# Fangjin98/distributed-training-INA

Hardware: AMD Instinct MI355X
Metric: aggregated-gradient GB/s (device-resident), 8-worker×100 MB int32 sum-reduce (higher is better)
Workload: dtype int32; 1 GPU; C3: 8 workers x 100 MiB int32 (26,214,400 values), V=256 slots; workers=8, slots=102400

## Files before the change

### distributed-training-ina_amd/csrc/ina_switch.hip

```cpp
#include <hip/hip_runtime.h>

#include <algorithm>
#include <atomic>
#include <cmath>
#include <mutex>
#include <unordered_map>

#include "ina.h"
#include "ina_internal.h"
#include "ina_device.h"

namespace ina {

using u32x4s = u32x4_t;
using f32x4s = f32x4_t;

constexpr int kSwBlock = 256;
constexpr int kMaxV = 256;
constexpr int kMaxStride = 16 + 4 * kMaxV;

__device__ __forceinline__ uint32_t from_next_lane(uint32_t x) {
    return (uint32_t)__builtin_amdgcn_update_dpp((int)x, (int)x, 0x130, 0xF, 0xF, false);
}
__device__ __forceinline__ uint32_t from_prev_lane(uint32_t x) {
// ... 614 lines not shown
#pragma unroll
    for (int o = 1; o < 64; o <<= 1) {
        const uint32_t y = (uint32_t)__shfl_up((int)x, o);
        if (lane >= o) x = max(x, y);
    }
    return x;
}
__device__ __forceinline__ uint32_t wave_suffix_min(uint32_t x) {
    const int lane = threadIdx.x & 63;
#pragma unroll
    for (int o = 1; o < 64; o <<= 1) {
        const uint32_t y = (uint32_t)__shfl_down((int)x, o);
        if (lane + o < 64) x = min(x, y);
    }
    return x;
}

#ifndef INA_LOC_TIMING
#define INA_LOC_TIMING 0
#endif
#if INA_LOC_TIMING
__device__ unsigned long long g_loc_t[8192][4];
#define LOC_STAMP(q) do { if (threadIdx.x == 0 && u < 8192) g_loc_t[u][q] = wall_clock64(); } while (0)
#define DEC_STAMP(row, q) do { if (threadIdx.x == 0) g_loc_t[row][q] = wall_clock64(); } while (0)
#else
#define LOC_STAMP(q) do { } while (0)
#define DEC_STAMP(row, q) do { } while (0)
#endif

struct LocUnit {
    uint32_t g_lo, lo, hi, pad;
};

__device__ __forceinline__ bool local_decide(const uint32_t* __restrict__ gmin, const uint32_t* __restrict__ gmax,
                                             uint32_t G, uint32_t gsize, size_t npk,
                                             uint32_t* __restrict__ unsorted, uint32_t epoch,
                                             LocUnit* __restrict__ units, bool writer, uint32_t* s_pm,
                                             uint32_t* s_sm, uint32_t* s_a, uint32_t* s_b) {
    __shared__ unsigned long long s_cost[kBkWaves];
    const int lane = threadIdx.x & 63, wv = wave_in_block();
    constexpr int kGpt = kLocMaxGran / kBkThr;
    const uint32_t kpt = (G + kBkThr - 1) / kBkThr;
    const uint32_t g0 = threadIdx.x * kpt;
    uint32_t pm[kGpt], sm[kGpt];
#pragma unroll
    for (int j = 0; j < kGpt; ++j) {
        const uint32_t g = g0 + (uint32_t)j;
        const bool ok = (uint32_t)j < kpt && g < G;
        pm[j] = ok ? gmax[g] : 0u;
        sm[j] = ok ? gmin[g] : 0xFFFFFFFFu;
    }
    uint32_t tmax = 0, tmin = 0xFFFFFFFFu;
#pragma unroll
    for (int j = 0; j < kGpt; ++j) pm[j] = tmax = max(tmax, pm[j]);
#pragma unroll
    for (int j = kGpt - 1; j >= 0; --j) sm[j] = tmin = min(tmin, sm[j]);
    const uint32_t imx = wave_incl_max(tmax), imn = wave_suffix_min(tmin);
    if (lane == 63) s_a[wv] = imx;
    if (lane == 0) s_b[wv] = imn;
    __syncthreads();
    uint32_t xmx = 0, xmn = 0xFFFFFFFFu, kmax = 0, kmin = 0xFFFFFFFFu;
#pragma unroll
    for (int w = 0; w < kBkWaves; ++w) {
        const uint32_t a = s_a[w], b = s_b[w];
        xmx = w < wv ? max(xmx, a) : xmx;
        xmn = w > wv ? min(xmn, b) : xmn;
        kmax = max(kmax, a);
        kmin = min(kmin, b);
    }
    {
        const uint32_t up = (uint32_t)__shfl_up((int)imx, 1), dn = (uint32_t)__shfl_down((int)imn, 1);
        if (lane > 0) xmx = max(xmx, up);
        if (lane < 63) xmn = min(xmn, dn);
    }
#pragma unroll
    for (int j = 0; j < kGpt; ++j) {
        const uint32_t g = g0 + (uint32_t)j;
        if ((uint32_t)j < kpt && g < G) {
            s_pm[g] = max(pm[j], xmx);
            s_sm[g] = min(sm[j], xmn);
        }
    }
    __syncthreads();
    if (kmin > kmax) return false;
    DEC_STAMP(8189, 0);
    constexpr uint32_t kUpt = (kLocMaxGran / kLocU + kBkThr - 1) / kBkThr;
    const uint32_t nu = (G + kLocU - 1) / kLocU;
    const uint32_t upt = (nu + kBkThr - 1) / kBkThr;
    LocUnit mu[kUpt];
    unsigned long long cost = 0;
    uint32_t maxwin = 0, glo = 0;
#pragma unroll
    for (uint32_t j = 0; j < kUpt; ++j) {
        const uint32_t u = threadIdx.x * upt + j;
        mu[j] = LocUnit{0u, 0u, 0u, 0u};
        if (j >= upt || u >= nu) continue;
        const uint32_t a = s_sm[u * kLocU];
        const uint32_t b = (u + 1) * kLocU < G ? s_sm[(u + 1) * kLocU] : 0xFFFFFFFFu;
        const uint32_t lo = a == 0xFFFFFFFFu ? kmax + 1u : a, hi = b == 0xFFFFFFFFu ? kmax + 1u : b;
        uint32_t l = glo, r = G;
        if (j > 0)
            for (int s = 0; s < 8 && l < r && s_pm[l] < lo; ++s) ++l;
        if (l < r && s_pm[l] < lo)
            while (l < r) {
                const uint32_t m = (l + r) >> 1;
                if (s_pm[m] >= lo) r = m; else l = m + 1;
            }
        glo = l;
        mu[j] = LocUnit{l, lo, hi, 0u};
        const size_t p0 = (size_t)l * gsize, p1 = min((size_t)(u + 1) * kLocU * gsize, npk);
        const uint32_t win = hi > lo && p1 > p0 ? (uint32_t)min(p1 - p0, (size_t)0xFFFFFFFFu) : 0u;
        cost += (unsigned long long)((hi - lo + kLlBins - 1) / kLlBins) * win;
        maxwin = max(maxwin, win);
    }
    DEC_STAMP(8189, 1);
#pragma unroll
    for (int o = 32; o > 0; o >>= 1) {
        cost += (unsigned long long)__shfl_xor((long long)cost, o);
        maxwin = max(maxwin, (uint32_t)__shfl_xor((int)maxwin, o));
    }
    if (lane == 0) {
        s_cost[wv] = cost;
        s_a[wv] = maxwin;
    }
    __syncthreads();
    unsigned long long total = 0;
    uint32_t mw = 0;
#pragma unroll
    for (int w = 0; w < kBkWaves; ++w) {
        total += s_cost[w];
        mw = max(mw, s_a[w]);
    }
    DEC_STAMP(8189, 2);
    if (mw > kLocMaxWindow || total > (unsigned long long)kLocBeta * npk) return false;
    if (writer) {
#pragma unroll
        for (uint32_t j = 0; j < kUpt; ++j) {
            const uint32_t u = threadIdx.x * upt + j;
            if (j < upt && u < nu) units[u] = mu[j];
        }
        if (threadIdx.x == 0) {
            unsorted[kLocKmin] = kmin;
            unsorted[kLocSlots] = kmax + 1u - kmin;
            unsorted[kLocUnits] = nu;
            unsorted[kLocEpoch] = epoch;
        }
    }
    return true;
}


__device__ __forceinline__ size_t switch_block_index();
__device__ __forceinline__ size_t xcd_block_index();
#ifndef INA_LL_WAVES_PER_EU
#define INA_LL_WAVES_PER_EU 8
#endif
__global__ __launch_bounds__(kLlWaves * 64) __attribute__((amdgpu_waves_per_eu(INA_LL_WAVES_PER_EU, 8))) void k_local_lists(const KeySrc keys_in, size_t npk,
                                                               uint32_t num_slots, uint32_t kmask,
                                                               const uint32_t* __restrict__ unsorted,
                                                               const LocUnit* __restrict__ units, uint32_t gsize,
                                                               uint32_t* __restrict__ ids, uint2* __restrict__ tab) {
    constexpr int kThr = kLlWaves * 64;
    constexpr int DPT = kLlBins / kThr;
    __shared__ uint32_t cw[kLlWaves / 2][kLlBins];
    __shared__ uint32_t s_ws[kLlWaves];
    const uint32_t ep = unsorted[1];
    if (unsorted[kLocEpoch] != ep) return;
    KeySrc kall = keys_in;
    kall.epoch = ep;
    const int lane = threadIdx.x & 63, wv = wave_in_block();
    const int sh = (wv & 1) * 16;
    uint32_t* crow = cw[wv >> 1];
    const unsigned long long below = (1ull << lane) - 1ull;
    const uint32_t kmin = unsorted[kLocKmin], nunits = unsorted[kLocUnits];
    for (uint32_t u = (uint32_t)xcd_block_index(); u < nunits; u += gridDim.x) {
        const LocUnit w = units[u];
        if (w.hi <= w.lo) continue;
        LOC_STAMP(0);
        const uint32_t P0 = w.g_lo * gsize, Pu = u * kLocU * gsize;
        const uint32_t P1 = (uint32_t)min((size_t)Pu + (size_t)kLocU * gsize, npk);
        const uint32_t per = ((P1 - P0 + kLlWaves * 64 - 1) / (kLlWaves * 64)) * 64;
        const uint32_t b0 = min(P0 + (uint32_t)wv * per, P1), b1 = min(b0 + per, P1);
        const bool held = per <= 64u * kLlRounds;
        KeySrc keys = kall;
        if (kall.desc && kall.flags) {
            bool miss = false;
            for (uint32_t f = (P0 >> kall.kb_shift) + (uint32_t)lane; f <= ((P1 - 1u) >> kall.kb_shift); f += 64u)
                miss |= kall.flags[f] != ep;
            if (__ballot(miss)) keys.flags = nullptr;
            else keys.desc = nullptr;
        }
        uint32_t kk[kLlRounds];
        if (held) {
#pragma unroll
            for (int r = 0; r < kLlRounds; ++r) {
                const uint32_t p = b0 + (uint32_t)(r * 64 + lane);
                kk[r] = p < b1 ? keys(p) : num_slots;
            }
        }
        uint32_t area = 0;
        for (uint32_t q = w.lo; q < w.hi; q += kLlBins) {
            const uint32_t qn = min((uint32_t)kLlBins, w.hi - q);
            for (uint32_t d = lane; d < (uint32_t)kLlBins; d += 64) crow[d] = 0u;
            __syncthreads();
            uint32_t before = 0;
            for (uint32_t r0 = b0; r0 < b1; r0 += 64 * kLlRounds) {
                if (!held) {
#pragma unroll
                    for (int r = 0; r < kLlRounds; ++r) {
                        const uint32_t p = r0 + (uint32_t)(r * 64 + lane);
                        kk[r] = p < b1 ? keys(p) : num_slots;
                    }
                }
#pragma unroll
                for (int r = 0; r < kLlRounds; ++r) {
                    const uint32_t slot = kk[r] & kmask;
                    const uint32_t p = r0 + (uint32_t)(r * 64 + lane);
                    lds_count_half(crow, slot - q, slot < num_slots && slot - q < qn, sh);
                    before += (p < Pu && p < b1 && (slot < w.lo || slot >= num_slots)) ? 1u : 0u;
                }
            }
            if (q == w.lo) {
#pragma unroll
                for (int o = 32; o > 0; o >>= 1) before += (uint32_t)__shfl_xor((int)before, o);
                if (lane == 0) s_ws[wv] = before;
            }
            __syncthreads();
            if (q == w.lo) {
                area = P0;
#pragma unroll
                for (int v = 0; v < kLlWaves; ++v) area += s_ws[v];
            }
            LOC_STAMP(1);
            uint32_t tc[DPT], tt = 0;
#pragma unroll
            for (int j = 0; j < DPT; ++j) {
                const uint32_t d = threadIdx.x * DPT + (uint32_t)j;
                uint32_t t = 0;
#pragma unroll
                for (int v2 = 0; v2 < kLlWaves / 2; ++v2) {
                    const uint32_t word = cw[v2][d];
                    t += (word & 0xFFFFu) + (word >> 16);
                }
                tc[j] = t;
                tt += t;
            }
            __syncthreads();
            const uint32_t inc = wave_incl_scan(tt);
            if (lane == 63) s_ws[wv] = inc;
            __syncthreads();
            uint32_t e = inc - tt, passn = 0;
#pragma unroll
            for (int v = 0; v < kLlWaves; ++v) {
                const uint32_t x = s_ws[v];
                e += v < wv ? x : 0u;
                passn += x;
            }
#pragma unroll
            for (int j = 0; j < DPT; ++j) {
                const uint32_t d = threadIdx.x * DPT + (uint32_t)j;
                if (d < qn) tab[q + d - kmin] = uint2{area + e, tc[j]};
                uint32_t b = e;
#pragma unroll
                for (int v2 = 0; v2 < kLlWaves / 2; ++v2) {
                    const uint32_t word = cw[v2][d];
                    const uint32_t lo16 = word & 0xFFFFu;
                    cw[v2][d] = b | ((b + lo16) << 16);
                    b += lo16 + (word >> 16);
                }
                e += tc[j];
            }
            __syncthreads();
            LOC_STAMP(2);
            for (uint32_t r0 = b0; r0 < b1; r0 += 64 * kLlRounds) {
                if (!held) {
#pragma unroll
                    for (int r = 0; r < kLlRounds; ++r) {
                        const uint32_t p = r0 + (uint32_t)(r * 64 + lane);
                        kk[r] = p < b1 ? keys(p) : num_slots;
                    }
                }
#pragma unroll
                for (int r = 0; r < kLlRounds; ++r) {
                    if (r0 + (uint32_t)(r * 64) >= b1) break;
                    const uint32_t slot = kk[r] & kmask;
                    const uint32_t d = slot - q;
                    const bool valid = slot < num_slots && d < qn;
                    const unsigned long long pm = lanes_with_digit(d, kLlBits, valid);
                    if (valid) {
                        const uint32_t rank = (uint32_t)__builtin_popcountll(pm & below);
                        const uint32_t cur = (crow[d] >> sh) & 0xFFFFu;
                        ids[area + cur + rank] = (r0 + (uint32_t)(r * 64 + lane)) | (kk[r] & ~kmask);
                        if (rank == 0) atomicAdd(&crow[d], (uint32_t)__builtin_popcountll(pm) << sh);
                    }
                }
            }
            area += passn;
            __syncthreads();
        }
        LOC_STAMP(3);
    }
}

#ifndef INA_SORT_STAGE_ALIAS
#define INA_SORT_STAGE_ALIAS 1
#endif
#ifndef INA_SORT_STAGE_MAX_R
#define INA_SORT_STAGE_MAX_R 8
#endif
#ifndef INA_SORT_STAGE
#define INA_SORT_STAGE 1
#endif
template <int R, int BINS, bool kStage = false, bool kPosOnly = false>
__device__ __forceinline__ void rs_tile_scatter_half(const uint32_t (&k)[R], const uint32_t (&v)[R],
                                                     size_t i0, size_t n, int shift, int bits,
                                                     uint32_t (*base)[BINS], const uint32_t* gst,
                                                     uint32_t* __restrict__ kout,
                                                     uint32_t* __restrict__ vout, int rw = R,
                                                     uint32_t* sk = nullptr, uint32_t* sv = nullptr,
                                                     uint32_t sbase = 0u, uint32_t* spos_out = nullptr) {
    const int lane = threadIdx.x & 63, wv = wave_in_block();
    const int sh = (wv & 1) * 16;
    uint32_t* row = base[wv >> 1];
    const uint32_t nb = 1u << bits;
    constexpr int kDPT = (BINS + kBkThr - 1) / kBkThr;
#pragma unroll
    for (int j = 0; j < kDPT; ++j) {
        const uint32_t d = threadIdx.x + (uint32_t)j * kBkThr;
        if (d >= nb) continue;
        uint32_t b = 0;
#pragma unroll
        for (int w2 = 0; w2 < kBkWaves / 2; ++w2) {
            const uint32_t word = base[w2][d];
            const uint32_t lo = word & 0xFFFFu, hi = word >> 16;
            base[w2][d] = b | ((b + lo) << 16);
            b += lo + hi;
        }
    }
    __syncthreads();
    const unsigned long long below = (1ull << lane) - 1ull;
    uint32_t spos[R];
#pragma unroll
    for (int r = 0; r < R; ++r) spos[r] = 0xFFFFFFFFu;
#pragma unroll
    for (int r = 0; r < R; ++r) {
        if (r >= rw || i0 - (size_t)lane + (size_t)r * 64 >= n) break;
        const bool valid = i0 + (size_t)r * 64 < n;
        const uint32_t d = (k[r] >> shift) & (nb - 1);
        const unsigned long long pm = lanes_with_digit(d, bits, valid);
        const uint32_t rank = (uint32_t)__builtin_popcountll(pm & below);
        const uint32_t b0 = (row[d] >> sh) & 0xFFFFu;
        if (valid) {
            const uint32_t pos = gst[d] + b0 + rank;
            if constexpr (kPosOnly) {
                spos[r] = pos - sbase;
            } else if constexpr (kStage) {
#if INA_SORT_STAGE_ALIAS
                spos[r] = pos - sbase;
#else
                sk[pos - sbase] = k[r];
                sv[pos - sbase] = v[r];
#endif
            } else {
                kout[pos] = k[r];
                vout[pos] = v[r];
            }
            if (rank == 0) atomicAdd(&row[d], (uint32_t)__builtin_popcountll(pm) << sh);
        }
    }
    if constexpr (kPosOnly) {
#pragma unroll
        for (int r = 0; r < R; ++r) spos_out[r] = spos[r];
        return;
    }
#if INA_SORT_STAGE_ALIAS
    if constexpr (kStage) {
        __syncthreads();
#pragma unroll
        for (int r = 0; r < R; ++r)
            if (spos[r] != 0xFFFFFFFFu) {
                sk[spos[r]] = k[r];
                sv[spos[r]] = v[r];
            }
    }
#endif
}

#ifndef INA_CHUNK_XCD
#define INA_CHUNK_XCD 1
#endif
#ifndef INA_BUCKET_STAGE
#define INA_BUCKET_STAGE 1
#endif
#ifndef INA_BUCKET_XCD
#define INA_BUCKET_XCD 0
#endif
#ifndef INA_BUCKET_GROUP
#define INA_BUCKET_GROUP 8
#endif
#ifndef INA_LAB_DETECT_NOACT
#define INA_LAB_DETECT_NOACT 0
#endif
template <int R, bool kDesc, int BINS, int kMode = 0>
__global__ __launch_bounds__(kBkThr) __attribute__((amdgpu_waves_per_eu(8, 8))) void k_sort_chunks(const uint8_t* __restrict__ pkts,
                                                        const uint2* __restrict__ desc, size_t npk,
                                                        size_t stride, uint32_t num_slots, int switch_id,
                                                        uint8_t* __restrict__ actions, int hbits, int lb,
                                                        uint32_t* __restrict__ rcnt, uint32_t* __restrict__ rst,
                                                        size_t nch, uint32_t* __restrict__ kout,
                                                        uint32_t* __restrict__ vout, int ack_hint,
                                                        uint32_t* __restrict__ unsorted, uint32_t epoch,
                                                        uint32_t* __restrict__ brk_cnt,
                                                        uint2* __restrict__ brk_ent,
                                                        uint32_t* __restrict__ gstat, LocUnit* __restrict__ units,
                                                        uint32_t decide_delay_ticks = 0,
                                                        uint32_t* __restrict__ kflags = nullptr,
                                                        const uint32_t* __restrict__ plain_hdr = nullptr) {
    constexpr bool kHalf = BINS > kBkThr;
    __shared__ uint32_t base[kHalf ? kBkWaves / 2 : kBkWaves][BINS];
    __shared__ uint32_t gst[BINS];
    __shared__ uint32_t wtot[kBkWaves];
    __shared__ uint32_t wbrk[kBkWaves];
    __shared__ uint32_t wgmn[kBkWaves], wgmx[kBkWaves];
    const int lane = threadIdx.x & 63, wv = wave_in_block();
    const size_t c = INA_CHUNK_XCD && kMode == 2 ? xcd_block_index() : blockIdx.x;
    const uint32_t G = (uint32_t)nch * (uint32_t)kGranPerChunk;
    if constexpr (kMode == 2) {
        if (unsorted[0] != epoch) return;
        if (c == 0) DEC_STAMP(8191, 0);
        if (c == nch - 1) DEC_STAMP(8190, 0);
        if (brk_cnt) {
            uint32_t part = 0;
            for (uint32_t cc = threadIdx.x; cc < (uint32_t)nch; cc += kBkThr) part += brk_cnt[cc];
            const uint32_t inc = wave_incl_scan(part);
            if (lane == 63) wtot[wv] = inc;
            __syncthreads();
            uint32_t total = 0;
#pragma unroll
            for (int w = 0; w < kBkWaves; ++w) total += wtot[w];
            __syncthreads();
            if (total <= (uint32_t)kRunsMax) {
                if (c == 0) build_run_table(brk_cnt, brk_ent, (uint32_t)nch, total, (uint32_t)npk, unsorted, epoch, wtot);
                return;
            }
        }
        if (gstat) {
            __shared__ uint32_t s_loc;
            unsigned long long* verdict = reinterpret_cast<unsigned long long*>(unsorted + kLocVerdict);
            if (c == 0) {
                DEC_STAMP(8191, 1);
                if (decide_delay_ticks) {
                    const unsigned long long t0 = wall_clock64();
                    while (wall_clock64() - t0 < decide_delay_ticks) __builtin_amdgcn_s_sleep(64);
                }
                const bool loc = local_decide(gstat, gstat + G, G, (uint32_t)(kBkThr * R / kGranPerChunk), npk,
                                              unsorted, epoch, units, true, &base[0][0],
                                              &base[0][0] + sizeof(base) / 8, wtot, wbrk);
                if (threadIdx.x == 0) {
                    __hip_atomic_store(verdict, ((unsigned long long)epoch << 1) | (loc ? 1ull : 0ull),
                                       __ATOMIC_RELAXED, __HIP_MEMORY_SCOPE_AGENT);
                    s_loc = loc ? 1u : 0u;
                }
                DEC_STAMP(8191, 2);
            } else if (threadIdx.x == 0) {
                unsigned long long v;
                uint32_t loc = 0u;
                const unsigned long long t0 = wall_clock64();
                for (;;) {
                    v = __hip_atomic_load(verdict, __ATOMIC_RELAXED, __HIP_MEMORY_SCOPE_AGENT);
                    if ((v >> 1) == epoch) {
                        loc = (uint32_t)(v & 1ull);
                        break;
                    }
                    if (wall_clock64() - t0 > kLocPollTicks) break;
                    __builtin_amdgcn_s_sleep(8);
                }
                s_loc = loc;
                if (c == nch - 1) DEC_STAMP(8190, 1);
            }
            __syncthreads();
            if (s_loc) return;
        }
    }
    const uint32_t nb = 1u << hbits;
    if constexpr (kMode != 1)
        for (uint32_t d = lane; d < nb; d += 64) base[kHalf ? wv >> 1 : wv][d] = 0;
    const size_t i0 = c * (size_t)(kBkThr * R) + (size_t)wv * (64 * R) + (size_t)lane;
    uint32_t idx[R], sid[R], ack[R], k[R], v[R];
    uint32_t plainm = 0u;
    if (kMode == 2 && plain_hdr) {
        const uint32_t w01 = plain_hdr[1], w02 = plain_hdr[2], w03 = plain_hdr[3];
        const uint32_t C0 = w01 & 0xFFu;
        const uint32_t B0 = __builtin_bswap32((w02 >> 24) | (w03 << 8)) - __builtin_bswap32((w01 >> 16) | (w02 << 16));
        if (c == 0 && threadIdx.x == 0) {
            unsorted[kPlainB] = B0;
            unsorted[kPlainC] = C0;
        }
#pragma unroll
        for (int r = 0; r < R; ++r) {
            const size_t p = i0 + (size_t)r * 64;
            uint32_t w1 = 0, w2 = 0, w3 = 0;
            if (p < npk) {
                const uint32_t* pk = plain_hdr + p * 4;
                w1 = pk[1];
                w2 = pk[2];
                w3 = pk[3];
            }
            idx[r] = __builtin_bswap32((w1 >> 16) | (w2 << 16));
            sid[r] = (w2 >> 16) & 0xFFu;
            ack[r] = (w1 >> 14) & 1u;
            const uint32_t fr = __builtin_bswap32((w2 >> 24) | (w3 << 8));
            const bool pl = (w1 & 0xFFFFu) == C0 && idx[r] < num_slots && fr - idx[r] == B0;
            plainm |= pl ? 1u << r : 0u;
        }
    } else {
        load_key_fields<R, kDesc>(pkts, desc, npk, stride, i0, idx, sid, ack);
    }
    uint32_t pidx[1], psid[1], pack[1];
    const size_t pw = i0 - (size_t)lane;
    load_key_fields<1, kDesc>(pkts, desc, pw > 0 ? npk : 0, stride, pw - 1, pidx, psid, pack);
    __syncthreads();
    const bool pmine = psid[0] == (uint32_t)(uint8_t)switch_id && switch_id >= 0;
    uint32_t prev = pmine ? pidx[0] % num_slots : num_slots;
    uint32_t prevf = prev | ((ack_hint && pmine && pack[0]) ? kAckBit : 0u);
    bool down = false;
    unsigned long long bm[R];
    uint32_t kmn = 0xFFFFFFFFu, kmx = 0u;
#pragma unroll
    for (int r = 0; r < R; ++r) {
        const size_t p = i0 + (size_t)r * 64;
        const bool mine = switch_id >= 0 && sid[r] == (uint32_t)(uint8_t)switch_id;
        const uint32_t key = mine ? idx[r] % num_slots : num_slots;
        if (kMode == 1 && mine && p < npk) {
            kmn = min(kmn, key);
            kmx = max(kmx, key);
        }
        k[r] = key | ((ack_hint && mine && ack[r]) ? kAckBit : 0u) | ((mine && ((plainm >> r) & 1u)) ? kPlainBit : 0u);
        v[r] = (uint32_t)p;
        if (kMode == 0 && p < npk && !mine) actions[p] = INA_ACT_FWD_OTHER;
        if (kMode == 1 && p < npk && !INA_LAB_DETECT_NOACT) actions[p] = mine ? INA_ACT_DROP : INA_ACT_FWD_OTHER;
        if constexpr (kMode != 1) {
            if constexpr (kHalf) lds_count_half(base[wv >> 1], (key >> lb) & (nb - 1), p < npk, (wv & 1) * 16);
            else lds_count(base[wv], (key >> lb) & (nb - 1), p < npk);
        }
        if constexpr (kMode == 1)
            if (p < npk && !kflags) kout[p] = k[r];
        const uint32_t pk = (uint32_t)__builtin_amdgcn_update_dpp((int)prev, (int)key, 0x138, 0xF, 0xF, false);
        down |= p < npk && p > 0 && pk > key;
        prev = (uint32_t)__builtin_amdgcn_readlane((int)key, 63);
        const uint32_t pkf = (uint32_t)__builtin_amdgcn_update_dpp((int)prevf, (int)k[r], 0x138, 0xF, 0xF, false);
        bm[r] = __ballot(p < npk && (p == 0 || !mine || (pkf & ~kAckBit) + 1u != key ||
                                     ((pkf ^ k[r]) & kAckBit) != 0u));
        prevf = (uint32_t)__builtin_amdgcn_readlane((int)k[r], 63);
    }
    if constexpr (kMode != 2) {
        if (__ballot(down) && lane == 0) unsorted[0] = epoch;
        if (c == 0 && threadIdx.x == 0) {
            unsorted[1] = epoch;
            unsorted[2] = 0u;
            unsorted[kLocEpoch] = 0u;
            unsorted[kLocVerdict] = 0u;
            unsorted[kLocVerdict + 1] = 0u;
        }
    }
    uint32_t nbw = 0;
#pragma unroll
    for (int r = 0; r < R; ++r) nbw += (uint32_t)__builtin_popcountll(bm[r]);
    if (lane == 0) wbrk[wv] = nbw;
    if (kMode == 1 && gstat) {
#pragma unroll
        for (int o = 32; o > 0; o >>= 1) {
            kmn = min(kmn, (uint32_t)__shfl_xor((int)kmn, o));
            kmx = max(kmx, (uint32_t)__shfl_xor((int)kmx, o));
        }
        if (lane == 0) {
            wgmn[wv] = kmn;
            wgmx[wv] = kmx;
        }
        if (kflags) {
            const bool st = __ballot(down) && kmx >= kmn && kmx - kmn <= kKeysSpanMax && kmx - kmn > kKeysSpanMin;
            if (st) {
#pragma unroll
                for (int r = 0; r < R; ++r)
                    if (i0 + (size_t)r * 64 < npk) kout[i0 + (size_t)r * 64] = k[r];
            }
            if (lane == 0) kflags[c * kBkWaves + wv] = st ? epoch : 0u;
        }
    }
    __syncthreads();
    if (kMode == 1 && gstat && threadIdx.x < (unsigned)kGranPerChunk) {
        uint32_t mn = 0xFFFFFFFFu, mx = 0u;
#pragma unroll
        for (int w = 0; w < kGranWaves; ++w) {
            mn = min(mn, wgmn[threadIdx.x * kGranWaves + w]);
            mx = max(mx, wgmx[threadIdx.x * kGranWaves + w]);
        }
        gstat[c * kGranPerChunk + threadIdx.x] = mn;
        gstat[G + c * kGranPerChunk + threadIdx.x] = mx;
    }
    if (kMode != 2 && brk_cnt) {
        uint32_t tot = 0, pre = 0;
#pragma unroll
        for (int w = 0; w < kBkWaves; ++w) {
            const uint32_t x = wbrk[w];
            tot += x;
            pre += w < wv ? x : 0u;
        }
        if (threadIdx.x == 0) brk_cnt[c] = tot;
        if (tot <= (uint32_t)kRunsMax && nbw) {
            const unsigned long long below = (1ull << lane) - 1ull;
#pragma unroll
            for (int r = 0; r < R; ++r) {
                if ((bm[r] >> lane) & 1ull)
                    brk_ent[c * kRunsMax + pre + (uint32_t)__builtin_popcountll(bm[r] & below)] =
                        uint2{(uint32_t)(i0 + (size_t)r * 64), k[r]};
                pre += (uint32_t)__builtin_popcountll(bm[r]);
            }
        }
    }
    if constexpr (kMode == 1) return;
    constexpr int DPT = kDigitsPerThread<BINS>;
    uint32_t tc[DPT], ex[DPT];
#pragma unroll
    for (int j = 0; j < DPT; ++j) {
        const uint32_t d = threadIdx.x * DPT + (uint32_t)j;
        tc[j] = 0;
        if (d < nb) {
            if constexpr (kHalf) {
#pragma unroll
                for (int w2 = 0; w2 < kBkWaves / 2; ++w2) {
                    const uint32_t word = base[w2][d];
                    tc[j] += (word & 0xFFFFu) + (word >> 16);
                }
            } else {
#pragma unroll
                for (int w = 0; w < kBkWaves; ++w) tc[j] += base[w][d];
            }
        }
    }
    block_digit_scan_n<DPT>(tc, ex, wtot, 0u);
#pragma unroll
    for (int j = 0; j < DPT; ++j) {
        const uint32_t d = threadIdx.x * DPT + (uint32_t)j;
        if (d < nb) {
            rcnt[(size_t)d * nch + c] = tc[j];
            rst[(size_t)d * nch + c] = ex[j];
            gst[d] = (uint32_t)(c * (size_t)(kBkThr * R)) + ex[j];
        }
    }
    __syncthreads();
#if INA_SORT_STAGE
    if constexpr (kHalf && R <= INA_SORT_STAGE_MAX_R) {
#if INA_SORT_STAGE_ALIAS
        static_assert(2 * kBkThr * R <= (kBkWaves / 2) * BINS, "staging fits the count array");
        uint32_t* s_k = &base[0][0];
        uint32_t* s_v = s_k + kBkThr * R;
#else
        __shared__ uint32_t s_k[kBkThr * R], s_v[kBkThr * R];
#endif
        const uint32_t cb = (uint32_t)(c * (size_t)(kBkThr * R));
        rs_tile_scatter_half<R, BINS, true>(k, v, i0, npk, lb, hbits, base, gst, kout, vout, R, s_k, s_v, cb);
        __syncthreads();
        const uint32_t nc = (uint32_t)min((size_t)(kBkThr * R), npk - (size_t)cb);
        for (uint32_t i = threadIdx.x; i < nc; i += kBkThr) {
            kout[cb + i] = s_k[i];
            vout[cb + i] = s_v[i];
        }
        return;
    }
#endif
    if constexpr (kHalf) rs_tile_scatter_half<R, BINS>(k, v, i0, npk, lb, hbits, base, gst, kout, vout);
    else rs_tile_scatter<R, kBkWaves, BINS>(k, v, i0, npk, lb, hbits, base, gst, kout, vout);
}

#ifndef INA_BK_TIMING
#define INA_BK_TIMING 0
#endif
#if INA_BK_TIMING
__device__ unsigned long long g_bk_t[kBkMaxChunks][6];
#define BK_STAMP(q) do { if (threadIdx.x == 0) g_bk_t[blockIdx.x][q] = wall_clock64(); } while (0)
#else
#define BK_STAMP(q) do { } while (0)
#endif

template <int R>
__device__ __forceinline__ void bucket_src(const uint32_t* s_dst, const uint32_t* s_src, uint32_t nch,
                                           uint32_t top, const uint32_t (&i)[R], uint32_t (&src)[R]) {
    uint32_t lo[R];
#pragma unroll
    for (int r = 0; r < R; ++r) lo[r] = 0;
    for (uint32_t step = top; step > 0; step >>= 1) {
#pragma unroll
        for (int r = 0; r < R; ++r) {
            const uint32_t t = lo[r] + step;
            if (t < nch && s_dst[t] <= i[r]) lo[r] = t;
        }
    }
#pragma unroll
    for (int r = 0; r < R; ++r) src[r] = s_src[lo[r]] + (i[r] - s_dst[lo[r]]);
}

template <int R, int BINS>
__global__ __launch_bounds__(kBkThr, BINS <= 1024 ? 2 * kBkThr / 256 : kBkThr / 256) void k_sort_buckets(const uint32_t* __restrict__ kin,
                                                         const uint32_t* __restrict__ vin,
                                                         uint32_t* __restrict__ kout,
                                                         uint32_t* __restrict__ vout,
                                                         const uint32_t* __restrict__ rcnt,
                                                         const uint32_t* __restrict__ rst, uint32_t nch,
                                                         uint32_t CH, int lbits, uint32_t* __restrict__ nforeign,
                                                         uint32_t skip, uint32_t* __restrict__ unsorted,
                                                         uint32_t epoch, int sorted_copy,
                                                         const uint32_t* __restrict__ brk_cnt,
                                                         const uint2* __restrict__ brk_ent, uint32_t npk,
                                                         int pre) {
    __shared__ uint32_t s_dst[kBkMaxChunks + 1], s_src[kBkMaxChunks];
    constexpr bool kHalf = BINS >= 1024;
    __shared__ uint32_t base[kHalf ? kBkWaves / 2 : kBkWaves][BINS];
    __shared__ uint32_t gst[BINS];
    __shared__ uint32_t red[kBkWaves], red2[kBkWaves];
    const int lane = threadIdx.x & 63, wv = wave_in_block();
    uint32_t b = INA_BUCKET_XCD ? (uint32_t)xcd_block_index() : blockIdx.x;
#if INA_BUCKET_GROUP > 1
    {
        constexpr uint32_t G = INA_BUCKET_GROUP;
        const uint32_t p = blockIdx.x, full = (gridDim.x / (8u * G)) * (8u * G);
        if (p < full) {
            const uint32_t x = p & 7u, i = p >> 3;
            b = (i / G) * (8u * G) + x * G + (i % G);
        }
    }
#endif
    const bool in_order = unsorted[0] != epoch;
    if (pre && (in_order || unsorted[2] == epoch || unsorted[kLocEpoch] == epoch)) return;
    if (in_order && !sorted_copy && b != skip) return;
    if (!in_order && brk_cnt) {
        uint32_t part = 0;
        for (uint32_t c = threadIdx.x; c < nch; c += kBkThr) part += brk_cnt[c];
        const uint32_t inc = wave_incl_scan(part);
        if (lane == 63) red[wv] = inc;
        __syncthreads();
        uint32_t total = 0;
#pragma unroll
        for (int w = 0; w < kBkWaves; ++w) total += red[w];
        if (total <= (uint32_t)kRunsMax) {
            if (b == 0) build_run_table(brk_cnt, brk_ent, nch, total, npk, unsorted, epoch, red2);
            return;
        }
        __syncthreads();
    }
    BK_STAMP(0);
    const uint32_t per = (nch + kBkThr - 1) / kBkThr;
    const uint32_t c0 = threadIdx.x * per;
    uint32_t part = 0, below = 0;
    for (uint32_t q = 0; q < per; ++q) {
        const uint32_t c = c0 + q;
        if (c < nch) {
            const uint32_t x = rcnt[(size_t)b * nch + c];
            const uint32_t st0 = rst[(size_t)b * nch + c];
            s_src[c] = c * CH + st0;
            s_dst[c] = x;
            part += x;
            below += st0;
        }
    }
    const uint32_t inc = wave_incl_scan(part);
    const uint32_t bsum = wave_incl_scan(below);
    if (lane == 63) {
        red[wv] = inc;
        red2[wv] = bsum;
    }
    __syncthreads();
    uint32_t wpre = 0, total = 0, s0 = 0;
#pragma unroll
    for (int w = 0; w < kBkWaves; ++w) {
        const uint32_t t = red[w];
        wpre += w < wv ? t : 0u;
        total += t;
        s0 += red2[w];
    }
    uint32_t run = wpre + inc - part;
    for (uint32_t q = 0; q < per; ++q) {
        const uint32_t c = c0 + q;
        if (c < nch) {
            const uint32_t x = s_dst[c];
            s_dst[c] = run;
            run += x;
        }
    }
    if (threadIdx.x == 0) s_dst[nch] = total;
    __syncthreads();
    BK_STAMP(1);
    const uint32_t cnt = total;
    if (b == skip) {
        if (threadIdx.x == 0) *nforeign = cnt;
        return;
    }
    if (cnt == 0) return;
    if (in_order) {
        for (uint32_t i = threadIdx.x; i < cnt; i += kBkThr) {
            kout[s0 + i] = kin[s0 + i];
            vout[s0 + i] = vin[s0 + i];
        }
        return;
    }
    uint32_t top = 1;
    while (top * 2 < nch) top *= 2;
    if (nch == 1) top = 0;
    if (lbits == 0) {
        for (uint32_t i0 = threadIdx.x; i0 - threadIdx.x < cnt; i0 += kBkThr) {
            const uint32_t ii[1] = {i0 < cnt ? i0 : 0u};
            uint32_t src[1];
            bucket_src<1>(s_dst, s_src, nch, top, ii, src);
            if (i0 < cnt) {
                kout[s0 + i0] = kin[src[0]];
                vout[s0 + i0] = vin[src[0]];
            }
        }
        return;
    }
    const uint32_t nb = 1u << lbits;
    constexpr int DPT = kDigitsPerThread<BINS>;
    for (uint32_t d = threadIdx.x; d < nb; d += kBkThr) gst[d] = 0;
    __syncthreads();
    constexpr uint32_t kTile = (uint32_t)kBkThr * (uint32_t)R;
    const uint32_t ntile = (cnt + kTile - 1) / kTile;
    if (ntile > 1) {
        for (uint32_t i = (uint32_t)wv * 64 + (uint32_t)lane; i - (uint32_t)lane < cnt; i += kBkThr) {
            const bool ok = i < cnt;
            const uint32_t ii[1] = {ok ? i : 0u};
            uint32_t src[1];
            bucket_src<1>(s_dst, s_src, nch, top, ii, src);
            lds_count(gst, ok ? kin[src[0]] & (nb - 1) : 0u, ok);
        }
        __syncthreads();
        uint32_t x[DPT], ex[DPT];
#pragma unroll
        for (int j = 0; j < DPT; ++j) {
            const uint32_t d = threadIdx.x * DPT + (uint32_t)j;
            x[j] = d < nb ? gst[d] : 0u;
        }
        block_digit_scan_n<DPT>(x, ex, red, s0);
#pragma unroll
        for (int j = 0; j < DPT; ++j) {
            const uint32_t d = threadIdx.x * DPT + (uint32_t)j;
            if (d < nb) gst[d] = ex[j];
        }
    }
    for (uint32_t t = 0; t < ntile; ++t) {
        const uint32_t tn = min(kTile, cnt - t * kTile);
        const int rw = (int)((tn + (uint32_t)kBkThr - 1) / (uint32_t)kBkThr);
        const uint32_t i0 = t * kTile + (uint32_t)wv * 64u * (uint32_t)rw + (uint32_t)lane;
        const uint32_t t_end = t * kTile + tn;
        uint32_t ii[R], src[R], k[R], v[R];
#pragma unroll
        for (int r = 0; r < R; ++r) {
            const uint32_t i = i0 + (uint32_t)r * 64u;
            ii[r] = (r < rw && i < t_end) ? i : 0u;
        }
        bucket_src<R>(s_dst, s_src, nch, top, ii, src);
#pragma unroll
        for (int r = 0; r < R; ++r) {
            const bool ok = r < rw && i0 + (uint32_t)r * 64u < t_end;
            k[r] = ok ? kin[src[r]] : 0u;
            v[r] = ok ? vin[src[r]] : 0u;
        }
        for (uint32_t dd = lane; dd < nb; dd += 64) base[kHalf ? wv >> 1 : wv][dd] = 0;
        __syncthreads();
#pragma unroll
        for (int r = 0; r < R; ++r)
            if (r < rw) {
                if constexpr (kHalf)
                    lds_count_half(base[wv >> 1], k[r] & (nb - 1), i0 + (uint32_t)r * 64u < t_end, (wv & 1) * 16);
                else
                    lds_count(base[wv], k[r] & (nb - 1), i0 + (uint32_t)r * 64u < t_end);
            }
        __syncthreads();
        BK_STAMP(2);
        uint32_t tc[DPT];
#pragma unroll
        for (int j = 0; j < DPT; ++j) {
            const uint32_t d = threadIdx.x * DPT + (uint32_t)j;
            tc[j] = 0;
            if (d < nb) {
                if constexpr (kHalf) {
#pragma unroll
                    for (int w2 = 0; w2 < kBkWaves / 2; ++w2) {
                        const uint32_t word = base[w2][d];
                        tc[j] += (word & 0xFFFFu) + (word >> 16);
                    }
                } else {
#pragma unroll
                    for (int w = 0; w < kBkWaves; ++w) tc[j] += base[w][d];
                }
            }
        }
        if (ntile == 1) {
            uint32_t ex[DPT];
            block_digit_scan_n<DPT>(tc, ex, red, s0);
#pragma unroll
            for (int j = 0; j < DPT; ++j) {
                const uint32_t d = threadIdx.x * DPT + (uint32_t)j;
                if (d < nb) gst[d] = ex[j];
            }
        }
        __syncthreads();
        BK_STAMP(3);
#if INA_BUCKET_STAGE
        if constexpr (kHalf) {
            if (ntile == 1) {
                static_assert((kBkWaves / 2) * BINS >= (int)kTile, "a tile fits the count array");
                uint32_t sp[R];
                rs_tile_scatter_half<R, BINS, false, true>(k, v, i0, t_end, 0, lbits, base, gst, kout, vout, rw,
                                                           nullptr, nullptr, s0, sp);
                uint32_t* stg = &base[0][0];
                __syncthreads();
#pragma unroll
                for (int r = 0; r < R; ++r)
                    if (sp[r] != 0xFFFFFFFFu) stg[sp[r]] = k[r];
                __syncthreads();
                for (uint32_t i = threadIdx.x; i < cnt; i += kBkThr) kout[s0 + i] = stg[i];
                __syncthreads();
#pragma unroll
                for (int r = 0; r < R; ++r)
                    if (sp[r] != 0xFFFFFFFFu) stg[sp[r]] = v[r];
                __syncthreads();
                for (uint32_t i = threadIdx.x; i < cnt; i += kBkThr) vout[s0 + i] = stg[i];
                return;
            }
        }
#endif
        if constexpr (kHalf) rs_tile_scatter_half<R, BINS>(k, v, i0, t_end, 0, lbits, base, gst, kout, vout, rw);
        else rs_tile_scatter<R, kBkWaves, BINS>(k, v, i0, t_end, 0, lbits, base, gst, kout, vout, rw);
        __syncthreads();
        BK_STAMP(4);
#pragma unroll
        for (int j = 0; j < DPT; ++j) {
            const uint32_t d = threadIdx.x * DPT + (uint32_t)j;
            if (d < nb) gst[d] += tc[j];
        }
    }
}

__global__ __launch_bounds__(kSwBlock) void k_switch_run(ina_switch_state_t st,
                                                         uint8_t* __restrict__ pkts, size_t npk,
                                                         size_t stride,
                                                         const uint32_t* __restrict__ keys,
                                                         const uint32_t* __restrict__ ids,
                                                         uint8_t* __restrict__ actions) {
    __shared__ __attribute__((aligned(16))) uint8_t stage[kSwBlock / 64][kMaxStride];
    const int lane = threadIdx.x & 63;
    const int wv = wave_in_block();
    const size_t pos = (size_t)blockIdx.x * (kSwBlock / 64) + wv;
    if (pos >= npk) return;
    const uint32_t slot = keys[pos];
    if (slot >= st.num_slots) return;
    if (pos > 0 && keys[pos - 1] == slot) return;
    const int V = st.V;
    uint8_t* lds = stage[wv];
    const bool vec = (stride % 16 == 0) && (((uintptr_t)pkts & 15u) == 0);
    const size_t span = stride < (size_t)kMaxStride ? stride : (size_t)kMaxStride;

    uint32_t cnt = st.count[slot];
    uint32_t frag = st.frag[slot];
    uint32_t reg[kMaxV / 64];
#pragma unroll
    for (int r = 0; r < kMaxV / 64; ++r) {
        int j = lane + 64 * r;
        reg[r] = j < V ? st.regs[(size_t)slot * V + j] : 0u;
    }

    for (size_t q = pos; q < npk && keys[q] == slot; ++q) {
        const uint32_t pid = ids[q];
        uint8_t* pk = pkts + (size_t)pid * stride;
        if (vec) {
            for (size_t b = 16 * (size_t)lane; b < span; b += 64 * 16)
                *reinterpret_cast<u32x4s*>(lds + b) = *reinterpret_cast<const u32x4s*>(pk + b);
        } else {
            for (size_t b = lane; b < span; b += 64) lds[b] = pk[b];
        }
        __builtin_amdgcn_wave_barrier();
        __builtin_amdgcn_fence(__ATOMIC_ACQUIRE, "wavefront");
        const uint32_t flags = lds[5];
        const uint32_t hcount = lds[4];
        const uint32_t frag_in = rd_be32(lds + 11);
        const bool is_ack = (flags >> 6) & 1u;
        uint8_t act;
        bool rewrite = false;
        if (is_ack) {
            frag = 0;
            act = INA_ACT_FWD_ACK;
        } else {
            if (frag == 0) frag = frag_in;
            if (frag != frag_in) {
                if (lane == 0) lds[5] = (uint8_t)(flags | INA_FLAG_COLLISION);
                act = INA_ACT_FWD_COLLISION;
                rewrite = true;
            } else {
                cnt = (cnt + 1u) & 0xFFu;
                if (cnt == hcount) cnt = 0;
                const bool first = (cnt == 1u);
#pragma unroll
                for (int r = 0; r < kMaxV / 64; ++r) {
                    int j = lane + 64 * r;
                    if (j < V) {
                        uint32_t lo = *reinterpret_cast<const uint32_t*>(lds + 12 + 4 * j);
                        uint32_t hi = *reinterpret_cast<const uint32_t*>(lds + 16 + 4 * j);
                        uint32_t v = __builtin_bswap32(__builtin_amdgcn_alignbyte(hi, lo, 3));
                        reg[r] = first ? v : reg[r] + v;
                    }
                }
                __builtin_amdgcn_wave_barrier();
#pragma unroll
                for (int r = 0; r < kMaxV / 64; ++r) {
                    int j = lane + 64 * r;
                    if (j < V) {
                        uint8_t* d = lds + 15 + 4 * j;
                        d[0] = (uint8_t)(reg[r] >> 24); d[1] = (uint8_t)(reg[r] >> 16);
                        d[2] = (uint8_t)(reg[r] >> 8);  d[3] = (uint8_t)reg[r];
                    }
                }
                act = cnt == 0 ? INA_ACT_FWD_AGG : INA_ACT_DROP;
                rewrite = act != INA_ACT_DROP || st.write_dropped;
            }
        }
        __builtin_amdgcn_wave_barrier();
        __builtin_amdgcn_fence(__ATOMIC_RELEASE, "wavefront");
        if (rewrite) {
            if (vec) {
                for (size_t b = 16 * (size_t)lane; b < span; b += 64 * 16)
                    *reinterpret_cast<u32x4s*>(pk + b) = *reinterpret_cast<const u32x4s*>(lds + b);
            } else {
                for (size_t b = lane; b < span; b += 64) pk[b] = lds[b];
            }
        }
        if (lane == 0) actions[pid] = act;
        __builtin_amdgcn_wave_barrier();
    }
    if (lane == 0) {
        st.count[slot] = (uint8_t)cnt;
        st.frag[slot] = frag;
    }
#pragma unroll
    for (int r = 0; r < kMaxV / 64; ++r) {
        int j = lane + 64 * r;
        if (j < V) st.regs[(size_t)slot * V + j] = reg[r];
    }
}


#ifndef INA_SWITCH_BATCH
#define INA_SWITCH_BATCH 8
#endif
constexpr int kB = INA_SWITCH_BATCH;
#ifndef INA_SWITCH_WIN_SMALL
#define INA_SWITCH_WIN_SMALL 8
#endif
#ifndef INA_SWITCH_WIN_NARROW
#define INA_SWITCH_WIN_NARROW 64
#endif
static_assert(INA_SWITCH_WIN_NARROW >= 1 && INA_SWITCH_WIN_NARROW <= 64, "a narrow window's heads are one wave's lanes");
#ifndef INA_SWITCH_WIN_LARGE
#define INA_SWITCH_WIN_LARGE 16
#endif
#ifndef INA_SWITCH_GRID
#define INA_SWITCH_GRID (1 << 20)
#endif
#ifndef INA_SWITCH_NARROW_SLOTS
#define INA_SWITCH_NARROW_SLOTS 1
#endif
static_assert(INA_SWITCH_WIN_SMALL >= 1 && INA_SWITCH_WIN_SMALL <= 64 && INA_SWITCH_WIN_LARGE >= 1 &&
              INA_SWITCH_WIN_LARGE <= 64, "a window is at most one wave of keys");
#ifndef INA_SWITCH_WAVES_RUN
#define INA_SWITCH_WAVES_RUN 7
#endif
#ifndef INA_SWITCH_WAVES
#define INA_SWITCH_WAVES 4
#endif

#ifndef INA_SWITCH_NT
#define INA_SWITCH_NT 1
#endif
#ifndef INA_SWITCH_TAIL_NT
#define INA_SWITCH_TAIL_NT 0
#endif
#ifndef INA_SWITCH_ACT_BATCH
#define INA_SWITCH_ACT_BATCH 1
#endif
__device__ __forceinline__ void sw_st(u32x4s v, u32x4s* p) {
#if INA_SWITCH_FWD_NT
    __builtin_nontemporal_store(v, p);
#else
    *p = v;
#endif
}
__device__ __forceinline__ u32x4s sw_ld(const u32x4s* p) {
#if INA_SWITCH_NT
    return __builtin_nontemporal_load(p);
#else
    return *p;
#endif
}

#ifndef INA_SWITCH_PERM
#define INA_SWITCH_PERM 1
#endif
__device__ __forceinline__ uint32_t dec_be(uint32_t hi, uint32_t lo) {
#if INA_SWITCH_PERM
    return __builtin_amdgcn_perm(hi, lo, 0x03040506u);
#else
    return __builtin_bswap32(__builtin_amdgcn_alignbyte(hi, lo, 3));
#endif
}
__device__ __forceinline__ uint32_t enc_lo(uint32_t prev, uint32_t v) {
#if INA_SWITCH_PERM
    return __builtin_amdgcn_perm(v, prev, 0x07000102u);
#else
    return (__builtin_bswap32(prev) >> 8) | (v & 0xFF000000u);
#endif
}

struct PsFuse {
    const float* local;
    float* out;
    size_t n;
    float inv, ws;
    uint32_t seq0, nslots;
    uint8_t* acks;
    size_t ack_stride;
    int on, keep_fwd;
    uint2* ack_desc;
};

template <bool kPs, bool kLat, bool kSplit, typename PidFn>
__device__ __forceinline__ void run_segment(const ina_switch_state_t& st, uint8_t* __restrict__ pkts,
                                            size_t stride, uint8_t* __restrict__ pay,
                                            uint8_t* __restrict__ actions, const PsFuse& ps,
                                            uint32_t slot, bool ack_led, size_t q_begin, size_t q_end,
                                            PidFn&& pid_batch, bool drop_written = false) {
    constexpr bool kActBatch = INA_SWITCH_ACT_BATCH;
    const int lane = threadIdx.x & 63;
    const int V = st.V;
    const int L = V >> 2;
    const bool vl = lane < L;
    const bool wide = L == 64;
    uint32_t cnt = 0, frag = 0, cnt_ld = 0, frag_ld = 0;
    bool st_ready = false;
    if constexpr (kLat) {
        cnt_ld = st.count[slot];
        frag_ld = st.frag[slot];
    } else {
        cnt = __builtin_amdgcn_readfirstlane((uint32_t)st.count[slot]);
        frag = ack_led ? 0u : __builtin_amdgcn_readfirstlane(st.frag[slot]);
    }
    u32x4s reg = {0u, 0u, 0u, 0u};
    bool have_reg = false;
    for (size_t q0 = q_begin; q0 < q_end; q0 += kB) {
        const int nb = (int)((q_end - q0) < (size_t)kB ? (q_end - q0) : (size_t)kB);
        u32x4s a[kB];
        uint32_t pid[kB];
        pid_batch(q0, nb, pid);
#pragma unroll
        for (int b = 1; b < kB; ++b) pid[b] = b < nb ? pid[b] : pid[0];
        u32x4s tl = {0u, 0u, 0u, 0u};
        uint32_t mypid = pid[0];
#pragma unroll
        for (int b = 1; b < kB; ++b) mypid = lane == b ? pid[b] : mypid;
        uint32_t act_v = 0;
        if constexpr (kSplit) {
            tl = *reinterpret_cast<const u32x4s*>(pkts + (size_t)mypid * 16);
#pragma unroll
            for (int b = 0; b < kB; ++b) {
                const u32x4s* pk = reinterpret_cast<const u32x4s*>(pay + (size_t)pid[b] * (size_t)(4 * V));
                a[b] = sw_ld(pk + (vl ? lane : 0));
            }
        } else {
        if (wide) {
#if INA_SWITCH_TAIL_NT
            tl = sw_ld(reinterpret_cast<const u32x4s*>(pkts + (size_t)mypid * stride) + 64);
#else
            tl = *(reinterpret_cast<const u32x4s*>(pkts + (size_t)mypid * stride) + 64);
#endif
        }
#pragma unroll
        for (int b = 0; b < kB; ++b) {
            const u32x4s* pk = reinterpret_cast<const u32x4s*>(pkts + (size_t)pid[b] * stride);
            a[b] = sw_ld(pk + (lane <= L ? lane : 0));
        }
        }
        if constexpr (kLat) {
            if (!st_ready) {
                cnt = __builtin_amdgcn_readfirstlane(cnt_ld);
                frag = ack_led ? 0u : __builtin_amdgcn_readfirstlane(frag_ld);
                st_ready = true;
            }
        }
#pragma unroll
        for (int b = 0; b < kB; ++b) {
            if (b >= nb) break;
            const uint32_t h1 = kSplit ? __builtin_amdgcn_readlane(tl.y, b) : __builtin_amdgcn_readlane(a[b].y, 0),
                           h2 = kSplit ? __builtin_amdgcn_readlane(tl.z, b) : __builtin_amdgcn_readlane(a[b].z, 0),
                           h3 = kSplit ? __builtin_amdgcn_readlane(tl.w, b) : __builtin_amdgcn_readlane(a[b].w, 0);
            const uint32_t hcount = h1 & 0xFFu, flags = (h1 >> 8) & 0xFFu;
            const uint32_t frag_in =
                __builtin_amdgcn_readfirstlane(__builtin_bswap32((h2 >> 24) | (h3 << 8)));
            uint8_t act;
            if ((flags >> 6) & 1u) {
                frag = 0;
                act = INA_ACT_FWD_ACK;
            } else {
                if (frag == 0) frag = frag_in;
                if (frag != frag_in) {
                    act = INA_ACT_FWD_COLLISION;
                    if (lane == 0)
                        reinterpret_cast<uint32_t*>(pkts + (size_t)pid[b] * (kSplit ? 16 : stride))[1] =
                            h1 | ((uint32_t)INA_FLAG_COLLISION << 8);
                } else {
// ... 1779 lines not shown
```

Measured before the change: 5652 GB/s.

## Pack in-chunk offset into sort key to drop value array in first pass

In the half-count bucket sort's first scatter pass, the value array is no longer written. Each key word now carries its hint bits, its low digit, and the element's offset within its chunk. The second (bucket) pass rebuilds the original key and the source id from that word and the bucket index, so it no longer reads the value array. This is meant to cut global memory traffic between the two passes roughly in half. It relies on the chunk size being a power of two and the packed fields fitting in one word, which is enforced with a static_assert.

```diff
diff --git a/distributed-training-ina_amd/csrc/ina_switch.hip b/distributed-training-ina_amd/csrc/ina_switch.hip
--- a/distributed-training-ina_amd/csrc/ina_switch.hip
+++ b/distributed-training-ina_amd/csrc/ina_switch.hip
@@ -940,22 +940,26 @@
     }
 }
 
-#ifndef INA_SORT_STAGE_ALIAS
-#define INA_SORT_STAGE_ALIAS 1
-#endif
-#ifndef INA_SORT_STAGE_MAX_R
-#define INA_SORT_STAGE_MAX_R 8
-#endif
 #ifndef INA_SORT_STAGE
 #define INA_SORT_STAGE 1
 #endif
-template <int R, int BINS, bool kStage = false, bool kPosOnly = false>
+constexpr uint32_t kSortHints = kAckBit | kPlainBit;
+template <int CH>
+constexpr bool kPackedFits = (CH & (CH - 1)) == 0 && (uint64_t)CH << kBitsBig <= (uint64_t)kPlainBit;
+__device__ __forceinline__ uint32_t sort_pack(uint32_t key, uint32_t off, int lb) {
+    return (key & kSortHints) | (off << lb) | (key & ((1u << lb) - 1u));
+}
+__device__ __forceinline__ void sort_unpack(uint32_t w, uint32_t src, uint32_t bucket, int lb, uint32_t chm,
+                                            uint32_t& key, uint32_t& id) {
+    key = (w & kSortHints) | (bucket << lb) | (w & ((1u << lb) - 1u));
+    id = (src & ~chm) | ((w & ~kSortHints) >> lb);
+}
+template <int R, int BINS, bool kPosOnly = false>
 __device__ __forceinline__ void rs_tile_scatter_half(const uint32_t (&k)[R], const uint32_t (&v)[R],
                                                      size_t i0, size_t n, int shift, int bits,
                                                      uint32_t (*base)[BINS], const uint32_t* gst,
                                                      uint32_t* __restrict__ kout,
                                                      uint32_t* __restrict__ vout, int rw = R,
-                                                     uint32_t* sk = nullptr, uint32_t* sv = nullptr,
                                                      uint32_t sbase = 0u, uint32_t* spos_out = nullptr) {
     const int lane = threadIdx.x & 63, wv = wave_in_block();
     const int sh = (wv & 1) * 16;
@@ -977,9 +981,10 @@
     }
     __syncthreads();
     const unsigned long long below = (1ull << lane) - 1ull;
-    uint32_t spos[R];
-#pragma unroll
-    for (int r = 0; r < R; ++r) spos[r] = 0xFFFFFFFFu;
+    if constexpr (kPosOnly) {
+#pragma unroll
+        for (int r = 0; r < R; ++r) spos_out[r] = 0xFFFFFFFFu;
+    }
 #pragma unroll
     for (int r = 0; r < R; ++r) {
         if (r >= rw || i0 - (size_t)lane + (size_t)r * 64 >= n) break;
@@ -991,14 +996,7 @@
         if (valid) {
             const uint32_t pos = gst[d] + b0 + rank;
             if constexpr (kPosOnly) {
-                spos[r] = pos - sbase;
-            } else if constexpr (kStage) {
-#if INA_SORT_STAGE_ALIAS
-                spos[r] = pos - sbase;
-#else
-                sk[pos - sbase] = k[r];
-                sv[pos - sbase] = v[r];
-#endif
+                spos_out[r] = pos - sbase;
             } else {
                 kout[pos] = k[r];
                 vout[pos] = v[r];
@@ -1006,22 +1004,6 @@
             if (rank == 0) atomicAdd(&row[d], (uint32_t)__builtin_popcountll(pm) << sh);
         }
     }
-    if constexpr (kPosOnly) {
-#pragma unroll
-        for (int r = 0; r < R; ++r) spos_out[r] = spos[r];
-        return;
-    }
-#if INA_SORT_STAGE_ALIAS
-    if constexpr (kStage) {
-        __syncthreads();
-#pragma unroll
-        for (int r = 0; r < R; ++r)
-            if (spos[r] != 0xFFFFFFFFu) {
-                sk[spos[r]] = k[r];
-                sv[spos[r]] = v[r];
-            }
-    }
-#endif
 }
 
 #ifndef INA_CHUNK_XCD
@@ -1287,28 +1269,29 @@
         }
     }
     __syncthreads();
+    if constexpr (kHalf) {
+        static_assert(kPackedFits<kBkThr * R>, "low digit + in-chunk offset + hint bits fit one word");
+        const uint32_t cb = (uint32_t)(c * (size_t)(kBkThr * R));
+        uint32_t sp[R];
+        rs_tile_scatter_half<R, BINS, true>(k, v, i0, npk, lb, hbits, base, gst, kout, vout, R, cb, sp);
 #if INA_SORT_STAGE
-    if constexpr (kHalf && R <= INA_SORT_STAGE_MAX_R) {
-#if INA_SORT_STAGE_ALIAS
-        static_assert(2 * kBkThr * R <= (kBkWaves / 2) * BINS, "staging fits the count array");
-        uint32_t* s_k = &base[0][0];
-        uint32_t* s_v = s_k + kBkThr * R;
-#else
-        __shared__ uint32_t s_k[kBkThr * R], s_v[kBkThr * R];
-#endif
-        const uint32_t cb = (uint32_t)(c * (size_t)(kBkThr * R));
-        rs_tile_scatter_half<R, BINS, true>(k, v, i0, npk, lb, hbits, base, gst, kout, vout, R, s_k, s_v, cb);
+        static_assert(kBkThr * R <= (kBkWaves / 2) * BINS, "staging fits the count array");
+        uint32_t* stg = &base[0][0];
+        __syncthreads();
+#pragma unroll
+        for (int r = 0; r < R; ++r)
+            if (sp[r] != 0xFFFFFFFFu) stg[sp[r]] = sort_pack(k[r], (uint32_t)(i0 + (size_t)r * 64) - cb, lb);
         __syncthreads();
         const uint32_t nc = (uint32_t)min((size_t)(kBkThr * R), npk - (size_t)cb);
-        for (uint32_t i = threadIdx.x; i < nc; i += kBkThr) {
-            kout[cb + i] = s_k[i];
-            vout[cb + i] = s_v[i];
-        }
-        return;
-    }
-#endif
-    if constexpr (kHalf) rs_tile_scatter_half<R, BINS>(k, v, i0, npk, lb, hbits, base, gst, kout, vout);
-    else rs_tile_scatter<R, kBkWaves, BINS>(k, v, i0, npk, lb, hbits, base, gst, kout, vout);
+        for (uint32_t i = threadIdx.x; i < nc; i += kBkThr) kout[cb + i] = stg[i];
+#else
+#pragma unroll
+        for (int r = 0; r < R; ++r)
+            if (sp[r] != 0xFFFFFFFFu) kout[cb + sp[r]] = sort_pack(k[r], (uint32_t)(i0 + (size_t)r * 64) - cb, lb);
+#endif
+    } else {
+        rs_tile_scatter<R, kBkWaves, BINS>(k, v, i0, npk, lb, hbits, base, gst, kout, vout);
+    }
 }
 
 #ifndef INA_BK_TIMING
@@ -1353,6 +1336,7 @@
                                                          int pre) {
     __shared__ uint32_t s_dst[kBkMaxChunks + 1], s_src[kBkMaxChunks];
     constexpr bool kHalf = BINS >= 1024;
+    constexpr bool kPacked = kHalf;
     __shared__ uint32_t base[kHalf ? kBkWaves / 2 : kBkWaves][BINS];
     __shared__ uint32_t gst[BINS];
     __shared__ uint32_t red[kBkWaves], red2[kBkWaves];
@@ -1436,8 +1420,11 @@
     if (cnt == 0) return;
     if (in_order) {
         for (uint32_t i = threadIdx.x; i < cnt; i += kBkThr) {
-            kout[s0 + i] = kin[s0 + i];
-            vout[s0 + i] = vin[s0 + i];
+            uint32_t kk = kin[s0 + i], vv;
+            if constexpr (kPacked) sort_unpack(kk, s0 + i, b, lbits, CH - 1u, kk, vv);
+            else vv = vin[s0 + i];
+            kout[s0 + i] = kk;
+            vout[s0 + i] = vv;
         }
         return;
     }
@@ -1450,8 +1437,11 @@
             uint32_t src[1];
             bucket_src<1>(s_dst, s_src, nch, top, ii, src);
             if (i0 < cnt) {
-                kout[s0 + i0] = kin[src[0]];
-                vout[s0 + i0] = vin[src[0]];
+                uint32_t kk = kin[src[0]], vv;
+                if constexpr (kPacked) sort_unpack(kk, src[0], b, lbits, CH - 1u, kk, vv);
+                else vv = vin[src[0]];
+                kout[s0 + i0] = kk;
+                vout[s0 + i0] = vv;
             }
         }
         return;
@@ -1500,7 +1490,8 @@
         for (int r = 0; r < R; ++r) {
             const bool ok = r < rw && i0 + (uint32_t)r * 64u < t_end;
             k[r] = ok ? kin[src[r]] : 0u;
-            v[r] = ok ? vin[src[r]] : 0u;
+            if constexpr (kPacked) sort_unpack(k[r], src[r], b, lbits, CH - 1u, k[r], v[r]);
+            else v[r] = ok ? vin[src[r]] : 0u;
         }
         for (uint32_t dd = lane; dd < nb; dd += 64) base[kHalf ? wv >> 1 : wv][dd] = 0;
         __syncthreads();
@@ -1548,8 +1539,7 @@
             if (ntile == 1) {
                 static_assert((kBkWaves / 2) * BINS >= (int)kTile, "a tile fits the count array");
                 uint32_t sp[R];
-                rs_tile_scatter_half<R, BINS, false, true>(k, v, i0, t_end, 0, lbits, base, gst, kout, vout, rw,
-                                                           nullptr, nullptr, s0, sp);
+                rs_tile_scatter_half<R, BINS, true>(k, v, i0, t_end, 0, lbits, base, gst, kout, vout, rw, s0, sp);
                 uint32_t* stg = &base[0][0];
                 __syncthreads();
 #pragma unroll
```

Measured after the change: 5614 GB/s (median of 3 runs). Within noise of the previous version (-0.7%).
